# microsoft/UniSpeech

Measured on NVIDIA H100. Metric: audio-sec/sec fwd+bwd, higher is better.
Workload: dtype bf16

## Files before the change

unispeech_b200/csrc/attn_fwd.cu:

```cuda
#include "../../include/unispeech_b200.h"
#include "attn_common.cuh"
#include "common.h"
#include <type_traits>

namespace b200 {

__device__ __forceinline__ float fast_exp2(float x) {
  float y;
  asm("ex2.approx.ftz.f32 %0, %1;" : "=f"(y) : "f"(x));
  return y;
}
__device__ __forceinline__ uint32_t warp_bit_transpose(uint32_t x, int lane) {
#pragma unroll
  for (int s = 16; s >= 1; s >>= 1) {
    const uint32_t m = (s == 16) ? 0x0000FFFFu : (s == 8) ? 0x00FF00FFu : (s == 4) ? 0x0F0F0F0Fu : (s == 2) ? 0x33333333u : 0x55555555u;
    const uint32_t y = __shfl_xor_sync(0xffffffffu, x, s);
    x = (lane & s) ? ((x & ~m) | ((y >> s) & m)) : ((x & m) | ((y << s) & ~m));
  }
  return x;
}
__device__ __forceinline__ void mbar_arrive_rel(uint64_t* bar) {
  asm volatile("mbarrier.arrive.release.cta.shared::cta.b64 _, [%0];" ::"r"(smem_u32(bar)) : "memory");
}

constexpr int kFwdQ = 0;
constexpr int kFwdK = 16384;
constexpr int kFwdV = 32768;
constexpr int kFwdP = 49152;
constexpr int kSPitch = kAttnTile + 4;
constexpr int kFwdS = 81920;
constexpr int kFwdStage = kFwdS + kAttnTile * kSPitch * 4;
constexpr int kFwdThreads = 160;
constexpr int kTabCopies = 4;
constexpr int kTabStride = 2 * kAttnTile + 8;
constexpr int kStageFloats = kTabCopies * kTabStride + kAttnTile + 4;
constexpr int kFwdSmem = kFwdStage + 2 * kStageFloats * 4 + 1024;
constexpr float kRebase = 1.2089258e24f;

__device__ __forceinline__ void lds_row32(const float* src, uint32_t* r) {
#pragma unroll
  for (int i = 0; i < 8; ++i) {
    const float4 v = reinterpret_cast<const float4*>(src)[i];
    r[4 * i] = __float_as_uint(v.x); r[4 * i + 1] = __float_as_uint(v.y);
    r[4 * i + 2] = __float_as_uint(v.z); r[4 * i + 3] = __float_as_uint(v.w);
  }
}

template <bool HAS_BIAS, bool DROP>
__global__ void __launch_bounds__(kFwdThreads, 1) attn_fwd_kernel(const __grid_constant__ CUtensorMap tm,
                                                                 const __grid_constant__ AttnParams p) {
  pdl_grid_sync();
  const int tid = threadIdx.x, warp = tid >> 5, lane = tid & 31;
  const int q0 = blockIdx.x * kAttnTile, h = blockIdx.y, b = blockIdx.z;
  const int T = p.T, D = p.D, N = p.n_tiles;

  extern __shared__ uint8_t smem_raw[];
  uint8_t* smem = smem_raw + ((1024u - (smem_u32(smem_raw) & 1023u)) & 1023u);
  uint8_t* sQ = smem + kFwdQ;
  uint8_t* sK = smem + kFwdK;
  uint8_t* sV = smem + kFwdV;
  uint8_t* sP = smem + kFwdP;
  float* s_f = reinterpret_cast<float*>(smem + kFwdS);
  float* stage = reinterpret_cast<float*>(smem + kFwdStage);

  __shared__ uint64_t q_full, k_full, k_empty, v_full, v_empty, stage_full[2];
  __shared__ float row_scale[kAttnTile];

  __shared__ int n_eff_s, live_s;
  if (tid == 0) { n_eff_s = p.key_pad != nullptr ? 1 : N; live_s = 0; }
  __syncthreads();
  if (p.key_pad != nullptr) {
    int last_valid = -1;
    bool live = false;
    for (int j = tid; j < T; j += kFwdThreads) {
      if (p.key_pad[static_cast<long long>(b) * T + j] == 0) {
        last_valid = j;
        if (j >= q0 && j < q0 + kAttnTile) live = true;
      }
    }
    if (last_valid >= 0) atomicMax(&n_eff_s, last_valid / kAttnTile + 1);
    if (live) live_s = 1;
  }
  __syncthreads();
  const int n_eff = n_eff_s;
  if (p.key_pad != nullptr && live_s == 0) {
    if (tid < kAttnTile && q0 + tid < T) {
      uint4* dst = reinterpret_cast<uint4*>(p.out + (static_cast<long long>(b) * T + q0 + tid) * D + h * kHeadDim);
#pragma unroll
      for (int g = 0; g < 8; ++g) dst[g] = make_uint4(0u, 0u, 0u, 0u);
      if (p.lse != nullptr) p.lse[(static_cast<long long>(b) * p.H + h) * T + q0 + tid] = INFINITY;
    }
    return;
  }

  if (warp == 4 && lane == 0) {
    tma_prefetch_desc(&tm);
    mbar_init(&q_full, 1);
    mbar_init(&k_full, 1);
    mbar_init(&v_full, 1);
    mbar_init(&k_empty, 4);
    mbar_init(&v_empty, 4);
    mbar_init(&stage_full[0], 32);
    mbar_init(&stage_full[1], 32);
    fence_mbar_init();
    mbar_expect_tx(&q_full, 16384);
    tma_load_4d(sQ, &tm, &q_full, h * kHeadDim, q0, b, 0);
    mbar_expect_tx(&k_full, 16384);
    tma_load_4d(sK, &tm, &k_full, D + h * kHeadDim, 0, b, 0);
    mbar_expect_tx(&v_full, 16384);
    tma_load_4d(sV, &tm, &v_full, 2 * D + h * kHeadDim, 0, b, 0);
  }
  __syncthreads();

  if (warp == 4) {
    auto fill_stage = [&](int n) {
      float* stg = stage + (n & 1) * kStageFloats;
      const int k0 = n * kAttnTile;
      if (HAS_BIAS) {
        const int base = k0 + (T - 1) - (q0 + kAttnTile - 1);
        const float* tab_h = p.tab + static_cast<long long>(h) * (2 * T - 1);
        float v[9];
#pragma unroll
        for (int t = 0; t < 9; ++t) {
          const int i = lane + 32 * t, gi = base + i;
          v[t] = (i < 2 * kAttnTile + kTabCopies - 1 && gi >= 0 && gi < 2 * T - 1) ? tab_h[gi] : 0.f;
        }
#pragma unroll
        for (int t = 0; t < 9; ++t)
#pragma unroll
          for (int c = 0; c < kTabCopies; ++c) {
            const int k = lane + 32 * t - c;
            if (k >= 0 && k < 2 * kAttnTile) stg[c * kTabStride + k] = v[t];
          }
      }
      float kb[4];
      int cnt = 0;
#pragma unroll
      for (int e = 0; e < 4; ++e) {
        const int j = k0 + 4 * lane + e;
        const bool masked = (j >= T) || (p.key_pad != nullptr && p.key_pad[static_cast<long long>(b) * T + j] != 0);
        kb[e] = masked ? -INFINITY : 0.f;
        cnt += masked ? 1 : 0;
      }
      reinterpret_cast<float4*>(stg + kTabCopies * kTabStride)[lane] = make_float4(kb[0], kb[1], kb[2], kb[3]);
      cnt = __reduce_add_sync(0xffffffffu, cnt);
      if (lane == 0) reinterpret_cast<int*>(stg)[kTabCopies * kTabStride + kAttnTile] = (cnt == 0) ? 0 : (cnt == kAttnTile ? 2 : 1);
      mbar_arrive(&stage_full[n & 1]);
    };
    fill_stage(0);
    if (n_eff > 1) fill_stage(1);
    for (int n = 1; n < n_eff; ++n) {
      const uint32_t ph = (n - 1) & 1;
      mbar_wait(&k_empty, ph);
      if (lane == 0) {
        mbar_expect_tx(&k_full, 16384);
        tma_load_4d(sK, &tm, &k_full, D + h * kHeadDim, n * kAttnTile, b, 0);
      }
      mbar_wait(&v_empty, ph);
      if (lane == 0) {
        mbar_expect_tx(&v_full, 16384);
        tma_load_4d(sV, &tm, &v_full, 2 * D + h * kHeadDim, n * kAttnTile, b, 0);
      }
      if (n + 1 < n_eff) fill_stage(n + 1);
    }
  } else {
    const int r = tid;
    const bool row_valid = (q0 + r) < T;
    const float* s_row = s_f + r * kSPitch;
    const int fr = 16 * (warp & 3) + (lane >> 2);
    float o_acc[2][32];

    float gl = 0.f;
    if (HAS_BIAS) {
      const float g = (p.gate != nullptr && row_valid) ? p.gate[(static_cast<long long>(b) * p.H + h) * T + q0 + r] : 1.0f;
      gl = g * kLog2e;
    }
    const float sc = p.scale * kLog2e;
    const int toff = kAttnTile - 1 - r;
    const int tab_off = (toff & 3) * kTabStride + (toff & ~3);
    uint32_t rk0 = 0, rk1 = 0;
    uint32_t* mask_row = nullptr;
    if (DROP) {
      const uint32_t rowid = static_cast<uint32_t>(b * p.H + h) * static_cast<uint32_t>(T) + static_cast<uint32_t>(q0 + r);
      rk0 = drop_row_k0(p.drop_k0, rowid);
      rk1 = drop_row_k1(p.drop_k1, rowid);
      mask_row = p.drop_mask + (static_cast<long long>(b * p.H + h) * (4 * N) + ((q0 + r) >> 5)) * (N * kAttnTile);
    }

    float m_ref = -INFINITY, l_run = 0.f;
    mbar_wait(&q_full, 0);

    for (int n = 0; n < n_eff; ++n) {
      const int k0 = n * kAttnTile;
      mbar_wait(&k_full, n & 1);
#pragma unroll 1
      for (int hm = 0; hm < 2; ++hm) {
        float acc[64];
        const uint32_t a = smem_u32(sQ) + hm * 8192, bb = smem_u32(sK);
        wgmma_fence();
#pragma unroll
        for (int k = 0; k < 4; ++k)
          wgmma_m64n128k16<0, 0>(acc, make_smem_desc_sw128(a + k * 32, 16, 1024), make_smem_desc_sw128(bb + k * 32, 16, 1024),
                                 k > 0 ? 1u : 0u);
        wgmma_commit();
        wgmma_wait<0>();
        acc_to_smem<128>(acc, s_f, kSPitch, 64 * hm);
      }
      if (lane == 0) mbar_arrive(&k_empty);
      named_bar_sync(1, kAttnTile);
      mbar_wait(&stage_full[n & 1], (n >> 1) & 1);
      const float* stg = stage + (n & 1) * kStageFloats;
      const float4* tab4 = reinterpret_cast<const float4*>(stg + tab_off);
      const float* kbias = stg + kTabCopies * kTabStride;
      const bool msk = reinterpret_cast<const int*>(stg)[kTabCopies * kTabStride + kAttnTile] != 0;

      auto tile_max = [&]() {
        float mx = -INFINITY;
#pragma unroll 1
        for (int c0 = 0; c0 < kAttnTile; c0 += 32) {
          uint32_t su[32];
          lds_row32(s_row + c0, su);
#pragma unroll
          for (int q = 0; q < 8; ++q) {
            float4 tb = make_float4(0.f, 0.f, 0.f, 0.f);
            if (HAS_BIAS) tb = tab4[c0 / 4 + q];
            float x0 = __uint_as_float(su[4 * q]) * sc, x1 = __uint_as_float(su[4 * q + 1]) * sc;
            float x2 = __uint_as_float(su[4 * q + 2]) * sc, x3 = __uint_as_float(su[4 * q + 3]) * sc;
            if (HAS_BIAS) {
              x0 = fmaf(gl, tb.x, x0); x1 = fmaf(gl, tb.y, x1); x2 = fmaf(gl, tb.z, x2); x3 = fmaf(gl, tb.w, x3);
            }
            if (msk) {
              const float4 kb = *reinterpret_cast<const float4*>(kbias + c0 + 4 * q);
              x0 += kb.x; x1 += kb.y; x2 += kb.z; x3 += kb.w;
            }
            mx = fmaxf(fmaxf(mx, fmaxf(x0, x1)), fmaxf(x2, x3));
          }
        }
        return mx;
      };

      if (__any_sync(0xffffffffu, m_ref == -INFINITY)) {
        const float mx = tile_max();
        if (m_ref == -INFINITY) m_ref = mx;
      }
      auto softmax_tile = [&](auto MSK) -> float {
        constexpr bool kMsk = decltype(MSK)::value;
        const float neg_ref = (m_ref == -INFINITY) ? 0.f : -m_ref;
        float part0 = 0.f, part1 = 0.f, part2 = 0.f, part3 = 0.f;
#pragma unroll 1
        for (int cc = 0; cc < 4; ++cc) {
          const int c0 = cc * 32;
          uint32_t su[32];
          lds_row32(s_row + c0, su);
          float pv[32];
          uint32_t rowbits = 0, hbits = 0;
#pragma unroll
          for (int q = 0; q < 8; ++q) {
            float4 tb = make_float4(0.f, 0.f, 0.f, 0.f), kb = make_float4(0.f, 0.f, 0.f, 0.f);
            if (HAS_BIAS) tb = tab4[c0 / 4 + q];
            if (kMsk) kb = *reinterpret_cast<const float4*>(kbias + c0 + 4 * q);
            const float tbv[4] = {tb.x, tb.y, tb.z, tb.w};
            const float kbv[4] = {kb.x, kb.y, kb.z, kb.w};
#pragma unroll
            for (int e = 0; e < 4; ++e) {
              const int j = 4 * q + e;
              float x = fmaf(__uint_as_float(su[j]), sc, neg_ref);
              if (HAS_BIAS) x = fmaf(gl, tbv[e], x);
              if (kMsk) x += kbv[e];
              const float ex = fast_exp2(x);
              if (e == 0) part0 += ex; else if (e == 1) part1 += ex; else if (e == 2) part2 += ex; else part3 += ex;
              if (DROP) {
                if ((j & 1) == 0) hbits = drop_bits(rk0, rk1, static_cast<uint32_t>(k0 + c0 + j) >> 1);
                const bool keep = (j & 1) ? drop_keep_hi(hbits, p.drop_thr_hi) : drop_keep_lo(hbits, p.drop_thr_hi);
                if (keep) rowbits |= (1u << j);
                pv[j] = keep ? ex : 0.f;
              } else {
                pv[j] = ex;
              }
            }
          }
          if (DROP) {
            const uint32_t mword = warp_bit_transpose(rowbits, lane);
            mask_row[k0 + c0 + lane] = mword;
          }
#pragma unroll
          for (int g = 0; g < 4; ++g) {
            uint4 w;
            w.x = pack_bf16x2(pv[g * 8 + 0], pv[g * 8 + 1]);
            w.y = pack_bf16x2(pv[g * 8 + 2], pv[g * 8 + 3]);
            w.z = pack_bf16x2(pv[g * 8 + 4], pv[g * 8 + 5]);
            w.w = pack_bf16x2(pv[g * 8 + 6], pv[g * 8 + 7]);
            store_sw128_chunk(sP, r, (c0 >> 3) + g, w);
          }
        }
        return (part0 + part1) + (part2 + part3);
      };
      float lsum, fac = 1.0f;
#pragma unroll 1
      while (true) {
        lsum = msk ? softmax_tile(std::true_type{}) : softmax_tile(std::false_type{});
        if (!__any_sync(0xffffffffu, !(lsum < kRebase))) break;
        const float m_new = fmaxf(m_ref, tile_max());
        const float factor = (m_ref == -INFINITY) ? 0.f : fast_exp2(m_ref - m_new);
        fac *= factor;
        l_run *= factor;
        m_ref = m_new;
      }
      l_run += lsum;
      row_scale[r] = fac;

      fence_proxy_async_smem();
      named_bar_sync(1, kAttnTile);
      if (n > 0) {
#pragma unroll
        for (int hm = 0; hm < 2; ++hm) {
          const float f0 = row_scale[64 * hm + fr], f1 = row_scale[64 * hm + fr + 8];
#pragma unroll
          for (int i = 0; i < 32; ++i) o_acc[hm][i] *= ((i >> 1) & 1) ? f1 : f0;
        }
      }
      mbar_wait(&v_full, n & 1);
      const uint32_t bv = smem_u32(sV);
      wgmma_fence();
#pragma unroll
      for (int hm = 0; hm < 2; ++hm) {
        const uint32_t a = smem_u32(sP) + hm * 8192;
#pragma unroll
        for (int k = 0; k < 8; ++k)
          wgmma_m64n64k16<0, 1>(o_acc[hm], make_smem_desc_sw128(a + (k >> 2) * 16384 + (k & 3) * 32, 16, 1024),
                                make_smem_desc_sw128(bv + k * 2048, 8192, 1024), (n > 0 || k > 0) ? 1u : 0u);
      }
      wgmma_commit();
      wgmma_wait<0>();
      if (lane == 0) mbar_arrive(&v_empty);
      named_bar_sync(1, kAttnTile);
    }

    row_scale[r] = l_run > 0.f ? (DROP ? p.drop_rp : 1.0f) / l_run : 0.f;
    if (row_valid && p.lse != nullptr)
      p.lse[(static_cast<long long>(b) * p.H + h) * T + q0 + r] = (l_run > 0.f) ? (m_ref + log2f(l_run)) : INFINITY;
    named_bar_sync(1, kAttnTile);
#pragma unroll
    for (int hm = 0; hm < 2; ++hm) {
#pragma unroll
      for (int rr = 0; rr < 2; ++rr) {
        const int row = 64 * hm + fr + 8 * rr;
        if (q0 + row < T) {
          const float inv = row_scale[row];
          __nv_bfloat16* dst = p.out + (static_cast<long long>(b) * T + q0 + row) * D + h * kHeadDim + 2 * (lane & 3);
#pragma unroll
          for (int g = 0; g < 8; ++g)
            *reinterpret_cast<uint32_t*>(dst + 8 * g) =
                pack_bf16x2(o_acc[hm][4 * g + 2 * rr] * inv, o_acc[hm][4 * g + 2 * rr + 1] * inv);
        }
      }
    }
  }
}

int make_qkv_tmap(CUtensorMap* out, const void* qkv, int T, int B, int D3, int box_rows);

}

using namespace b200;

extern "C" {

int b200s_attn_fwd_dropout(const void* qkv, const float* gate, const float* tab, const uint8_t* key_pad, void* out, float* lse,
                           int B, int T, int H, float scale, float drop_p, uint32_t key0, uint32_t key1, uint32_t* drop_mask,
                           b200s_stream stream) {
  B200_CHECK_ARG(qkv && out, "attn_fwd: null pointer");
  B200_CHECK_ARG(drop_p >= 0.f && drop_p < 1.f, "attn_fwd: dropout p=%f out of range [0,1)", static_cast<double>(drop_p));
  B200_CHECK_ARG(drop_p == 0.f || drop_mask != nullptr, "attn_fwd: dropout needs the mask buffer (b200s_attn_dropout_mask_words)");
  B200_CHECK_ARG(static_cast<long long>(B) * H * T < (1LL << 32), "attn_fwd: B*H*T exceeds the 32-bit dropout row counter");
  const int D = H * kHeadDim;
  CUtensorMap tm;
  AttnParams p;
  memset(&p, 0, sizeof(p));
  p.T = T; p.H = H; p.B = B; p.D = D;
  p.n_tiles = ceil_div(T, kAttnTile);
  B200_CHECK_ARG(T >= 1, "attn_fwd: T=%d out of range", T);
  const int smem = kFwdSmem;
  if (make_qkv_tmap(&tm, qkv, T, B, 3 * D, kAttnTile)) return -3;
  p.scale = scale;
  p.gate = gate; p.tab = tab; p.key_pad = key_pad;
  p.out = static_cast<__nv_bfloat16*>(out);
  p.lse = lse;
  const bool drop = drop_p > 0.f;
  p.drop_mask = drop_mask;
  p.drop_k0 = key0; p.drop_k1 = key1;
  p.drop_thr_hi = drop_threshold16(drop_p) << 16;
  p.drop_rp = 1.0f / (1.0f - drop_p);
  dim3 grid(ceil_div(T, kAttnTile), H, B);
  cudaStream_t st = static_cast<cudaStream_t>(stream);
  void (*kern)(const CUtensorMap, const AttnParams) =
      tab != nullptr ? (drop ? attn_fwd_kernel<true, true> : attn_fwd_kernel<true, false>)
                     : (drop ? attn_fwd_kernel<false, true> : attn_fwd_kernel<false, false>);
  B200_CHECK_CUDA(cudaFuncSetAttribute(kern, cudaFuncAttributeMaxDynamicSharedMemorySize, smem));
  B200_CHECK_CUDA(launch_pdl(kern, dim3(grid), dim3(kFwdThreads), smem, st, tm, p));
  B200_CHECK_LAUNCH();
  return 0;
}

int b200s_attn_fwd(const void* qkv, const float* gate, const float* tab, const uint8_t* key_pad, void* out, float* lse,
                   int B, int T, int H, float scale, b200s_stream stream) {
  return b200s_attn_fwd_dropout(qkv, gate, tab, key_pad, out, lse, B, T, H, scale, 0.f, 0u, 0u, nullptr, stream);
}

long long b200s_attn_dropout_mask_words(int B, int T, int H) { return attn_drop_mask_words(B, H, T); }

}
```

Before: 2505.

## Restructure attention forward into two warpgroups with register softmax and pipelined QK/PV

Replaces the one-warpgroup-plus-producer-warp design with two consumer warpgroups of 128 threads, each owning 64 query rows. The S tile stays in registers instead of round-tripping through shared memory, and P is fed to the PV wgmma from registers. A three-stage K/V TMA ring lets the QK^T of tile n overlap the PV of tile n-1, and bias and mask staging move to per-warpgroup cp.async. This removes the smem S/P traffic and the serialised wgmma waits, at the cost of higher register pressure and a more complex rebase path that recomputes S when the running sum overflows.

```diff
diff --git a/unispeech_b200/csrc/attn_fwd.cu b/unispeech_b200/csrc/attn_fwd.cu
--- a/unispeech_b200/csrc/attn_fwd.cu
+++ b/unispeech_b200/csrc/attn_fwd.cu
@@ -19,32 +19,37 @@
   }
   return x;
 }
-__device__ __forceinline__ void mbar_arrive_rel(uint64_t* bar) {
-  asm volatile("mbarrier.arrive.release.cta.shared::cta.b64 _, [%0];" ::"r"(smem_u32(bar)) : "memory");
-}
-
+__device__ __forceinline__ uint32_t compact_every4(uint32_t x) {
+  x &= 0x11111111u;
+  x = (x | (x >> 3)) & 0x03030303u;
+  x = (x | (x >> 6)) & 0x000F000Fu;
+  return (x | (x >> 12)) & 0xFFu;
+}
+__device__ __forceinline__ bool named_bar_any(int id, int count, bool pred) {
+  uint32_t r;
+  asm volatile(
+      "{\n\t.reg .pred p, q;\n\t"
+      "setp.ne.u32 p, %1, 0;\n\t"
+      "bar.red.or.pred q, %2, %3, p;\n\t"
+      "selp.u32 %0, 1, 0, q;\n\t}"
+      : "=r"(r)
+      : "r"(static_cast<uint32_t>(pred)), "r"(id), "r"(count)
+      : "memory");
+  return r != 0;
+}
+
+constexpr int kFwdStages = 3;
 constexpr int kFwdQ = 0;
 constexpr int kFwdK = 16384;
-constexpr int kFwdV = 32768;
-constexpr int kFwdP = 49152;
-constexpr int kSPitch = kAttnTile + 4;
-constexpr int kFwdS = 81920;
-constexpr int kFwdStage = kFwdS + kAttnTile * kSPitch * 4;
-constexpr int kFwdThreads = 160;
-constexpr int kTabCopies = 4;
-constexpr int kTabStride = 2 * kAttnTile + 8;
-constexpr int kStageFloats = kTabCopies * kTabStride + kAttnTile + 4;
-constexpr int kFwdSmem = kFwdStage + 2 * kStageFloats * 4 + 1024;
+constexpr int kFwdV = kFwdK + kFwdStages * 16384;
+constexpr int kFwdStage = kFwdV + kFwdStages * 16384;
+constexpr int kFwdThreads = 256;
+constexpr int kTabCopies = 2;
+constexpr int kWgWin = 192;
+constexpr int kTabStride = kWgWin + 8;
+constexpr int kStageFloats = kTabCopies * kTabStride + kAttnTile;
+constexpr int kFwdSmem = kFwdStage + 4 * kStageFloats * 4 + 1024;
 constexpr float kRebase = 1.2089258e24f;
-
-__device__ __forceinline__ void lds_row32(const float* src, uint32_t* r) {
-#pragma unroll
-  for (int i = 0; i < 8; ++i) {
-    const float4 v = reinterpret_cast<const float4*>(src)[i];
-    r[4 * i] = __float_as_uint(v.x); r[4 * i + 1] = __float_as_uint(v.y);
-    r[4 * i + 2] = __float_as_uint(v.z); r[4 * i + 3] = __float_as_uint(v.w);
-  }
-}
 
 template <bool HAS_BIAS, bool DROP>
 __global__ void __launch_bounds__(kFwdThreads, 1) attn_fwd_kernel(const __grid_constant__ CUtensorMap tm,
@@ -59,12 +64,9 @@
   uint8_t* sQ = smem + kFwdQ;
   uint8_t* sK = smem + kFwdK;
   uint8_t* sV = smem + kFwdV;
-  uint8_t* sP = smem + kFwdP;
-  float* s_f = reinterpret_cast<float*>(smem + kFwdS);
   float* stage = reinterpret_cast<float*>(smem + kFwdStage);
 
-  __shared__ uint64_t q_full, k_full, k_empty, v_full, v_empty, stage_full[2];
-  __shared__ float row_scale[kAttnTile];
+  __shared__ uint64_t q_full, k_full[kFwdStages], k_empty[kFwdStages], v_full[kFwdStages], v_empty[kFwdStages];
 
   __shared__ int n_eff_s, live_s;
   if (tid == 0) { n_eff_s = p.key_pad != nullptr ? 1 : N; live_s = 0; }
@@ -93,268 +95,284 @@
     return;
   }
 
-  if (warp == 4 && lane == 0) {
+  if (tid == 0) {
     tma_prefetch_desc(&tm);
     mbar_init(&q_full, 1);
-    mbar_init(&k_full, 1);
-    mbar_init(&v_full, 1);
-    mbar_init(&k_empty, 4);
-    mbar_init(&v_empty, 4);
-    mbar_init(&stage_full[0], 32);
-    mbar_init(&stage_full[1], 32);
+#pragma unroll
+    for (int s = 0; s < kFwdStages; ++s) {
+      mbar_init(&k_full[s], 1);
+      mbar_init(&v_full[s], 1);
+      mbar_init(&k_empty[s], 8);
+      mbar_init(&v_empty[s], 8);
+    }
     fence_mbar_init();
     mbar_expect_tx(&q_full, 16384);
     tma_load_4d(sQ, &tm, &q_full, h * kHeadDim, q0, b, 0);
-    mbar_expect_tx(&k_full, 16384);
-    tma_load_4d(sK, &tm, &k_full, D + h * kHeadDim, 0, b, 0);
-    mbar_expect_tx(&v_full, 16384);
-    tma_load_4d(sV, &tm, &v_full, 2 * D + h * kHeadDim, 0, b, 0);
+    for (int n = 0; n < 2 && n < n_eff; ++n) {
+      mbar_expect_tx(&k_full[n], 16384);
+      tma_load_4d(sK + n * 16384, &tm, &k_full[n], D + h * kHeadDim, n * kAttnTile, b, 0);
+      mbar_expect_tx(&v_full[n], 16384);
+      tma_load_4d(sV + n * 16384, &tm, &v_full[n], 2 * D + h * kHeadDim, n * kAttnTile, b, 0);
+    }
   }
   __syncthreads();
 
-  if (warp == 4) {
-    auto fill_stage = [&](int n) {
-      float* stg = stage + (n & 1) * kStageFloats;
-      const int k0 = n * kAttnTile;
-      if (HAS_BIAS) {
-        const int base = k0 + (T - 1) - (q0 + kAttnTile - 1);
-        const float* tab_h = p.tab + static_cast<long long>(h) * (2 * T - 1);
-        float v[9];
-#pragma unroll
-        for (int t = 0; t < 9; ++t) {
-          const int i = lane + 32 * t, gi = base + i;
-          v[t] = (i < 2 * kAttnTile + kTabCopies - 1 && gi >= 0 && gi < 2 * T - 1) ? tab_h[gi] : 0.f;
+  const int c = warp >> 2, w = warp & 3, qd = lane & 3;
+  const int r0 = 64 * c + 16 * w + (lane >> 2);
+  const float sc = p.scale * kLog2e;
+  float gl[2] = {0.f, 0.f};
+  uint32_t rk0[2] = {0u, 0u}, rk1[2] = {0u, 0u};
+#pragma unroll
+  for (int hh = 0; hh < 2; ++hh) {
+    const int row = q0 + r0 + 8 * hh;
+    if (HAS_BIAS) {
+      const float g = (p.gate != nullptr && row < T) ? p.gate[(static_cast<long long>(b) * p.H + h) * T + row] : 1.0f;
+      gl[hh] = g * kLog2e;
+    }
+    if (DROP) {
+      const uint32_t rowid = static_cast<uint32_t>(b * p.H + h) * static_cast<uint32_t>(T) + static_cast<uint32_t>(row);
+      rk0[hh] = drop_row_k0(p.drop_k0, rowid);
+      rk1[hh] = drop_row_k1(p.drop_k1, rowid);
+    }
+  }
+  float* const wg_stage = stage + 2 * c * kStageFloats;
+  const int t = tid & 127;
+  const float* tab_h = HAS_BIAS ? p.tab + static_cast<long long>(h) * (2 * T - 1) : nullptr;
+  auto fill_bias = [&](int n) {
+    float* stg = wg_stage + (n & 1) * kStageFloats;
+    const int gbase = n * kAttnTile + T - 64 - 64 * c - q0;
+#pragma unroll
+    for (int u = 0; u < 3; ++u) {
+      const int e = (t + 128 * u) / kWgWin, i = (t + 128 * u) % kWgWin, gi = gbase + i + e;
+      const bool ok = gi >= 0 && gi < 2 * T - 1;
+      cp_async_4_zfill(stg + e * kTabStride + i, tab_h + (ok ? gi : 0), ok);
+    }
+    cp_async_commit();
+  };
+  auto key_masked = [&](int n) {
+    const int j = n * kAttnTile + t;
+    return j >= T || (p.key_pad != nullptr && p.key_pad[static_cast<long long>(b) * T + j] != 0);
+  };
+  const int tbase = 63 + 64 * c - r0 + 2 * qd;
+  const int tab_off = (tbase & 1) * kTabStride + (tbase & ~1);
+  uint16_t* mask_half = nullptr;
+  if (DROP)
+    mask_half = reinterpret_cast<uint16_t*>(p.drop_mask + (static_cast<long long>(b * p.H + h) * (4 * N) + (q0 >> 5) + 2 * c + (w >> 1)) *
+                                                              (N * kAttnTile)) + (w & 1);
+
+  float s[64];
+  float o[32];
+  uint32_t pr[32];
+#pragma unroll
+  for (int i = 0; i < 32; ++i) o[i] = 0.f;
+  float m_ref[2] = {-INFINITY, -INFINITY}, l_run[2] = {0.f, 0.f};
+  const uint32_t qa = smem_u32(sQ) + c * 8192;
+
+  auto issue_s = [&](int n) {
+    const uint32_t kb = smem_u32(sK) + (n % kFwdStages) * 16384;
+#pragma unroll
+    for (int k = 0; k < 4; ++k)
+      wgmma_m64n128k16<0, 0>(s, make_smem_desc_sw128(qa + k * 32, 16, 1024), make_smem_desc_sw128(kb + k * 32, 16, 1024),
+                             k > 0 ? 1u : 0u);
+  };
+  auto issue_pv = [&](int n) {
+    const uint32_t vb = smem_u32(sV) + (n % kFwdStages) * 16384;
+#pragma unroll
+    for (int k = 0; k < 8; ++k) wgmma_m64n64k16_rs<1>(o, pr + 4 * k, make_smem_desc_sw128(vb + k * 2048, 8192, 1024), 1u);
+  };
+
+  auto refill = [&](int n, uint64_t* empty, uint64_t* full, uint8_t* ring, int col) {
+    if (tid == 0 && n + 2 < n_eff) {
+      const int slot = (n + 2) % kFwdStages;
+      if (n > 0) mbar_wait(&empty[slot], ((n - 1) / kFwdStages) & 1);
+      mbar_expect_tx(&full[slot], 16384);
+      tma_load_4d(ring + slot * 16384, &tm, &full[slot], col + h * kHeadDim, (n + 2) * kAttnTile, b, 0);
+    }
+  };
+  float o_fac[2] = {1.f, 1.f};
+  bool rebased = false;
+  bool km = false;
+  auto softmax_step = [&](int n) {
+    const int k0 = n * kAttnTile;
+    if (HAS_BIAS) cp_async_wait_all();
+    const bool msk = named_bar_any(1 + c, 128, km);
+    bool km_next = false;
+    if (n + 1 < n_eff) {
+      if (HAS_BIAS) fill_bias(n + 1);
+      km_next = key_masked(n + 1);
+    }
+    const float* stg = wg_stage + (n & 1) * kStageFloats;
+    const float* tabp = stg + tab_off;
+    const float* kbias = stg + kTabCopies * kTabStride + 2 * qd;
+
+    auto tile_max = [&](float (&mx)[2]) {
+      mx[0] = mx[1] = -INFINITY;
+#pragma unroll
+      for (int g = 0; g < 16; ++g) {
+        const float2 kb = msk ? *reinterpret_cast<const float2*>(kbias + 8 * g) : make_float2(0.f, 0.f);
+#pragma unroll
+        for (int hh = 0; hh < 2; ++hh) {
+          float2 tb = make_float2(0.f, 0.f);
+          if (HAS_BIAS) tb = *reinterpret_cast<const float2*>(tabp + 8 * (g - hh));
+          float x0 = s[4 * g + 2 * hh] * sc, x1 = s[4 * g + 2 * hh + 1] * sc;
+          if (HAS_BIAS) { x0 = fmaf(gl[hh], tb.x, x0); x1 = fmaf(gl[hh], tb.y, x1); }
+          if (msk) { x0 += kb.x; x1 += kb.y; }
+          mx[hh] = fmaxf(mx[hh], fmaxf(x0, x1));
         }
-#pragma unroll
-        for (int t = 0; t < 9; ++t)
-#pragma unroll
-          for (int c = 0; c < kTabCopies; ++c) {
-            const int k = lane + 32 * t - c;
-            if (k >= 0 && k < 2 * kAttnTile) stg[c * kTabStride + k] = v[t];
-          }
-      }
-      float kb[4];
-      int cnt = 0;
-#pragma unroll
-      for (int e = 0; e < 4; ++e) {
-        const int j = k0 + 4 * lane + e;
-        const bool masked = (j >= T) || (p.key_pad != nullptr && p.key_pad[static_cast<long long>(b) * T + j] != 0);
-        kb[e] = masked ? -INFINITY : 0.f;
-        cnt += masked ? 1 : 0;
-      }
-      reinterpret_cast<float4*>(stg + kTabCopies * kTabStride)[lane] = make_float4(kb[0], kb[1], kb[2], kb[3]);
-      cnt = __reduce_add_sync(0xffffffffu, cnt);
-      if (lane == 0) reinterpret_cast<int*>(stg)[kTabCopies * kTabStride + kAttnTile] = (cnt == 0) ? 0 : (cnt == kAttnTile ? 2 : 1);
-      mbar_arrive(&stage_full[n & 1]);
+      }
+#pragma unroll
+      for (int hh = 0; hh < 2; ++hh) {
+        mx[hh] = fmaxf(mx[hh], __shfl_xor_sync(0xffffffffu, mx[hh], 1));
+        mx[hh] = fmaxf(mx[hh], __shfl_xor_sync(0xffffffffu, mx[hh], 2));
+      }
     };
-    fill_stage(0);
-    if (n_eff > 1) fill_stage(1);
-    for (int n = 1; n < n_eff; ++n) {
-      const uint32_t ph = (n - 1) & 1;
-      mbar_wait(&k_empty, ph);
-      if (lane == 0) {
-        mbar_expect_tx(&k_full, 16384);
-        tma_load_4d(sK, &tm, &k_full, D + h * kHeadDim, n * kAttnTile, b, 0);
-      }
-      mbar_wait(&v_empty, ph);
-      if (lane == 0) {
-        mbar_expect_tx(&v_full, 16384);
-        tma_load_4d(sV, &tm, &v_full, 2 * D + h * kHeadDim, n * kAttnTile, b, 0);
-      }
-      if (n + 1 < n_eff) fill_stage(n + 1);
-    }
-  } else {
-    const int r = tid;
-    const bool row_valid = (q0 + r) < T;
-    const float* s_row = s_f + r * kSPitch;
-    const int fr = 16 * (warp & 3) + (lane >> 2);
-    float o_acc[2][32];
-
-    float gl = 0.f;
-    if (HAS_BIAS) {
-      const float g = (p.gate != nullptr && row_valid) ? p.gate[(static_cast<long long>(b) * p.H + h) * T + q0 + r] : 1.0f;
-      gl = g * kLog2e;
-    }
-    const float sc = p.scale * kLog2e;
-    const int toff = kAttnTile - 1 - r;
-    const int tab_off = (toff & 3) * kTabStride + (toff & ~3);
-    uint32_t rk0 = 0, rk1 = 0;
-    uint32_t* mask_row = nullptr;
-    if (DROP) {
-      const uint32_t rowid = static_cast<uint32_t>(b * p.H + h) * static_cast<uint32_t>(T) + static_cast<uint32_t>(q0 + r);
-      rk0 = drop_row_k0(p.drop_k0, rowid);
-      rk1 = drop_row_k1(p.drop_k1, rowid);
-      mask_row = p.drop_mask + (static_cast<long long>(b * p.H + h) * (4 * N) + ((q0 + r) >> 5)) * (N * kAttnTile);
-    }
-
-    float m_ref = -INFINITY, l_run = 0.f;
-    mbar_wait(&q_full, 0);
-
-    for (int n = 0; n < n_eff; ++n) {
-      const int k0 = n * kAttnTile;
-      mbar_wait(&k_full, n & 1);
-#pragma unroll 1
-      for (int hm = 0; hm < 2; ++hm) {
-        float acc[64];
-        const uint32_t a = smem_u32(sQ) + hm * 8192, bb = smem_u32(sK);
-        wgmma_fence();
-#pragma unroll
-        for (int k = 0; k < 4; ++k)
-          wgmma_m64n128k16<0, 0>(acc, make_smem_desc_sw128(a + k * 32, 16, 1024), make_smem_desc_sw128(bb + k * 32, 16, 1024),
-                                 k > 0 ? 1u : 0u);
-        wgmma_commit();
-        wgmma_wait<0>();
-        acc_to_smem<128>(acc, s_f, kSPitch, 64 * hm);
-      }
-      if (lane == 0) mbar_arrive(&k_empty);
-      named_bar_sync(1, kAttnTile);
-      mbar_wait(&stage_full[n & 1], (n >> 1) & 1);
-      const float* stg = stage + (n & 1) * kStageFloats;
-      const float4* tab4 = reinterpret_cast<const float4*>(stg + tab_off);
-      const float* kbias = stg + kTabCopies * kTabStride;
-      const bool msk = reinterpret_cast<const int*>(stg)[kTabCopies * kTabStride + kAttnTile] != 0;
-
-      auto tile_max = [&]() {
-        float mx = -INFINITY;
-#pragma unroll 1
-        for (int c0 = 0; c0 < kAttnTile; c0 += 32) {
-          uint32_t su[32];
-          lds_row32(s_row + c0, su);
-#pragma unroll
-          for (int q = 0; q < 8; ++q) {
-            float4 tb = make_float4(0.f, 0.f, 0.f, 0.f);
-            if (HAS_BIAS) tb = tab4[c0 / 4 + q];
-            float x0 = __uint_as_float(su[4 * q]) * sc, x1 = __uint_as_float(su[4 * q + 1]) * sc;
-            float x2 = __uint_as_float(su[4 * q + 2]) * sc, x3 = __uint_as_float(su[4 * q + 3]) * sc;
-            if (HAS_BIAS) {
-              x0 = fmaf(gl, tb.x, x0); x1 = fmaf(gl, tb.y, x1); x2 = fmaf(gl, tb.z, x2); x3 = fmaf(gl, tb.w, x3);
+    if (__any_sync(0xffffffffu, m_ref[0] == -INFINITY || m_ref[1] == -INFINITY)) {
+      float mx[2];
+      tile_max(mx);
+#pragma unroll
+      for (int hh = 0; hh < 2; ++hh)
+        if (m_ref[hh] == -INFINITY) m_ref[hh] = mx[hh];
+    }
+    uint32_t rowbits[2];
+    auto softmax_tile = [&](auto MSK, float (&lsum)[2]) {
+      constexpr bool kMsk = decltype(MSK)::value;
+      float part[2][2] = {{0.f, 0.f}, {0.f, 0.f}};
+      rowbits[0] = rowbits[1] = 0u;
+#pragma unroll
+      for (int g = 0; g < 16; ++g) {
+        float2 kb = make_float2(0.f, 0.f);
+        if (kMsk) kb = *reinterpret_cast<const float2*>(kbias + 8 * g);
+#pragma unroll
+        for (int hh = 0; hh < 2; ++hh) {
+          const float neg_ref = (m_ref[hh] == -INFINITY) ? 0.f : -m_ref[hh];
+          float2 tb = make_float2(0.f, 0.f);
+          if (HAS_BIAS) tb = *reinterpret_cast<const float2*>(tabp + 8 * (g - hh));
+          const float tbv[2] = {tb.x, tb.y}, kbv[2] = {kb.x, kb.y};
+          uint32_t hbits = 0u;
+          if (DROP) hbits = drop_bits(rk0[hh], rk1[hh], static_cast<uint32_t>(k0 + 8 * g + 2 * qd) >> 1);
+#pragma unroll
+          for (int e = 0; e < 2; ++e) {
+            const int i = 4 * g + 2 * hh + e;
+            float x = fmaf(s[i], sc, neg_ref);
+            if (HAS_BIAS) x = fmaf(gl[hh], tbv[e], x);
+            if (kMsk) x += kbv[e];
+            const float ex = fast_exp2(x);
+            part[hh][e] += ex;
+            if (DROP) {
+              const bool keep = e ? drop_keep_hi(hbits, p.drop_thr_hi) : drop_keep_lo(hbits, p.drop_thr_hi);
+              if (keep) rowbits[hh] |= 1u << (2 * g + e);
+              s[i] = keep ? ex : 0.f;
+            } else {
+              s[i] = ex;
             }
-            if (msk) {
-              const float4 kb = *reinterpret_cast<const float4*>(kbias + c0 + 4 * q);
-              x0 += kb.x; x1 += kb.y; x2 += kb.z; x3 += kb.w;
-            }
-            mx = fmaxf(fmaxf(mx, fmaxf(x0, x1)), fmaxf(x2, x3));
           }
         }
-        return mx;
-      };
-
-      if (__any_sync(0xffffffffu, m_ref == -INFINITY)) {
-        const float mx = tile_max();
-        if (m_ref == -INFINITY) m_ref = mx;
-      }
-      auto softmax_tile = [&](auto MSK) -> float {
-        constexpr bool kMsk = decltype(MSK)::value;
-        const float neg_ref = (m_ref == -INFINITY) ? 0.f : -m_ref;
-        float part0 = 0.f, part1 = 0.f, part2 = 0.f, part3 = 0.f;
-#pragma unroll 1
-        for (int cc = 0; cc < 4; ++cc) {
-          const int c0 = cc * 32;
-          uint32_t su[32];
-          lds_row32(s_row + c0, su);
-          float pv[32];
-          uint32_t rowbits = 0, hbits = 0;
-#pragma unroll
-          for (int q = 0; q < 8; ++q) {
-            float4 tb = make_float4(0.f, 0.f, 0.f, 0.f), kb = make_float4(0.f, 0.f, 0.f, 0.f);
-            if (HAS_BIAS) tb = tab4[c0 / 4 + q];
-            if (kMsk) kb = *reinterpret_cast<const float4*>(kbias + c0 + 4 * q);
-            const float tbv[4] = {tb.x, tb.y, tb.z, tb.w};
-            const float kbv[4] = {kb.x, kb.y, kb.z, kb.w};
-#pragma unroll
-            for (int e = 0; e < 4; ++e) {
-              const int j = 4 * q + e;
-              float x = fmaf(__uint_as_float(su[j]), sc, neg_ref);
-              if (HAS_BIAS) x = fmaf(gl, tbv[e], x);
-              if (kMsk) x += kbv[e];
-              const float ex = fast_exp2(x);
-              if (e == 0) part0 += ex; else if (e == 1) part1 += ex; else if (e == 2) part2 += ex; else part3 += ex;
-              if (DROP) {
-                if ((j & 1) == 0) hbits = drop_bits(rk0, rk1, static_cast<uint32_t>(k0 + c0 + j) >> 1);
-                const bool keep = (j & 1) ? drop_keep_hi(hbits, p.drop_thr_hi) : drop_keep_lo(hbits, p.drop_thr_hi);
-                if (keep) rowbits |= (1u << j);
-                pv[j] = keep ? ex : 0.f;
-              } else {
-                pv[j] = ex;
-              }
-            }
-          }
-          if (DROP) {
-            const uint32_t mword = warp_bit_transpose(rowbits, lane);
-            mask_row[k0 + c0 + lane] = mword;
-          }
-#pragma unroll
-          for (int g = 0; g < 4; ++g) {
-            uint4 w;
-            w.x = pack_bf16x2(pv[g * 8 + 0], pv[g * 8 + 1]);
-            w.y = pack_bf16x2(pv[g * 8 + 2], pv[g * 8 + 3]);
-            w.z = pack_bf16x2(pv[g * 8 + 4], pv[g * 8 + 5]);
-            w.w = pack_bf16x2(pv[g * 8 + 6], pv[g * 8 + 7]);
-            store_sw128_chunk(sP, r, (c0 >> 3) + g, w);
-          }
-        }
-        return (part0 + part1) + (part2 + part3);
-      };
-      float lsum, fac = 1.0f;
-#pragma unroll 1
-      while (true) {
-        lsum = msk ? softmax_tile(std::true_type{}) : softmax_tile(std::false_type{});
-        if (!__any_sync(0xffffffffu, !(lsum < kRebase))) break;
-        const float m_new = fmaxf(m_ref, tile_max());
-        const float factor = (m_ref == -INFINITY) ? 0.f : fast_exp2(m_ref - m_new);
-        fac *= factor;
-        l_run *= factor;
-        m_ref = m_new;
-      }
-      l_run += lsum;
-      row_scale[r] = fac;
-
-      fence_proxy_async_smem();
-      named_bar_sync(1, kAttnTile);
-      if (n > 0) {
-#pragma unroll
-        for (int hm = 0; hm < 2; ++hm) {
-          const float f0 = row_scale[64 * hm + fr], f1 = row_scale[64 * hm + fr + 8];
-#pragma unroll
-          for (int i = 0; i < 32; ++i) o_acc[hm][i] *= ((i >> 1) & 1) ? f1 : f0;
-        }
-      }
-      mbar_wait(&v_full, n & 1);
-      const uint32_t bv = smem_u32(sV);
+      }
+#pragma unroll
+      for (int hh = 0; hh < 2; ++hh) {
+        float v = part[hh][0] + part[hh][1];
+        v += __shfl_xor_sync(0xffffffffu, v, 1);
+        v += __shfl_xor_sync(0xffffffffu, v, 2);
+        lsum[hh] = v;
+      }
+    };
+    float lsum[2];
+    if (msk) softmax_tile(std::true_type{}, lsum); else softmax_tile(std::false_type{}, lsum);
+    bool need[2] = {!(lsum[0] < kRebase), !(lsum[1] < kRebase)};
+    if (named_bar_any(1 + c, 128, need[0] || need[1])) {
+      wgmma_wait<0>();
       wgmma_fence();
-#pragma unroll
-      for (int hm = 0; hm < 2; ++hm) {
-        const uint32_t a = smem_u32(sP) + hm * 8192;
-#pragma unroll
-        for (int k = 0; k < 8; ++k)
-          wgmma_m64n64k16<0, 1>(o_acc[hm], make_smem_desc_sw128(a + (k >> 2) * 16384 + (k & 3) * 32, 16, 1024),
-                                make_smem_desc_sw128(bv + k * 2048, 8192, 1024), (n > 0 || k > 0) ? 1u : 0u);
-      }
+      issue_s(n);
       wgmma_commit();
       wgmma_wait<0>();
-      if (lane == 0) mbar_arrive(&v_empty);
-      named_bar_sync(1, kAttnTile);
-    }
-
-    row_scale[r] = l_run > 0.f ? (DROP ? p.drop_rp : 1.0f) / l_run : 0.f;
-    if (row_valid && p.lse != nullptr)
-      p.lse[(static_cast<long long>(b) * p.H + h) * T + q0 + r] = (l_run > 0.f) ? (m_ref + log2f(l_run)) : INFINITY;
-    named_bar_sync(1, kAttnTile);
-#pragma unroll
-    for (int hm = 0; hm < 2; ++hm) {
-#pragma unroll
-      for (int rr = 0; rr < 2; ++rr) {
-        const int row = 64 * hm + fr + 8 * rr;
-        if (q0 + row < T) {
-          const float inv = row_scale[row];
-          __nv_bfloat16* dst = p.out + (static_cast<long long>(b) * T + q0 + row) * D + h * kHeadDim + 2 * (lane & 3);
-#pragma unroll
-          for (int g = 0; g < 8; ++g)
-            *reinterpret_cast<uint32_t*>(dst + 8 * g) =
-                pack_bf16x2(o_acc[hm][4 * g + 2 * rr] * inv, o_acc[hm][4 * g + 2 * rr + 1] * inv);
-        }
-      }
-    }
+      float mx[2];
+      tile_max(mx);
+      rebased = true;
+#pragma unroll
+      for (int hh = 0; hh < 2; ++hh) {
+        if (!need[hh]) continue;
+        const float m_new = fmaxf(m_ref[hh], mx[hh]);
+        const float factor = (m_ref[hh] == -INFINITY) ? 0.f : fast_exp2(m_ref[hh] - m_new);
+        l_run[hh] *= factor;
+        o_fac[hh] = factor;
+        m_ref[hh] = m_new;
+      }
+      if (msk) softmax_tile(std::true_type{}, lsum); else softmax_tile(std::false_type{}, lsum);
+    }
+    l_run[0] += lsum[0];
+    l_run[1] += lsum[1];
+    if (lane == 0) mbar_arrive(&k_empty[n % kFwdStages]);
+    refill(n, k_empty, k_full, sK, D);
+
+    if (DROP) {
+      const uint32_t t0 = warp_bit_transpose(rowbits[0], lane), t1 = warp_bit_transpose(rowbits[1], lane);
+      const int col = k0 + 8 * (lane >> 1) + (lane & 1);
+#pragma unroll
+      for (int q = 0; q < 4; ++q)
+        mask_half[2 * (col + 2 * q)] = static_cast<uint16_t>(compact_every4(t0 >> q) | (compact_every4(t1 >> q) << 8));
+    }
+    if (n + 1 < n_eff) wg_stage[((n + 1) & 1) * kStageFloats + kTabCopies * kTabStride + t] = km_next ? -INFINITY : 0.f;
+    km = km_next;
+  };
+  auto apply_rebase = [&]() {
+    if (rebased) {
+#pragma unroll
+      for (int i = 0; i < 32; ++i) o[i] *= o_fac[(i >> 1) & 1];
+      o_fac[0] = o_fac[1] = 1.f;
+      rebased = false;
+    }
+  };
+  auto pack_p = [&]() {
+#pragma unroll
+    for (int m = 0; m < 32; ++m) pr[m] = pack_bf16x2(s[2 * m], s[2 * m + 1]);
+  };
+
+  if (HAS_BIAS) fill_bias(0);
+  km = key_masked(0);
+  wg_stage[kTabCopies * kTabStride + t] = km ? -INFINITY : 0.f;
+  mbar_wait(&q_full, 0);
+  mbar_wait(&k_full[0], 0);
+  wgmma_fence();
+  issue_s(0);
+  wgmma_commit();
+  wgmma_wait<0>();
+  softmax_step(0);
+  refill(0, v_empty, v_full, sV, 2 * D);
+  apply_rebase();
+  pack_p();
+  for (int n = 1; n < n_eff; ++n) {
+    mbar_wait(&k_full[n % kFwdStages], (n / kFwdStages) & 1);
+    mbar_wait(&v_full[(n - 1) % kFwdStages], ((n - 1) / kFwdStages) & 1);
+    wgmma_fence();
+    issue_s(n);
+    wgmma_commit();
+    issue_pv(n - 1);
+    wgmma_commit();
+    wgmma_wait<1>();
+    softmax_step(n);
+    wgmma_wait<0>();
+    if (lane == 0) mbar_arrive(&v_empty[(n - 1) % kFwdStages]);
+    refill(n, v_empty, v_full, sV, 2 * D);
+    apply_rebase();
+    pack_p();
+  }
+  mbar_wait(&v_full[(n_eff - 1) % kFwdStages], ((n_eff - 1) / kFwdStages) & 1);
+  wgmma_fence();
+  issue_pv(n_eff - 1);
+  wgmma_commit();
+  wgmma_wait<0>();
+
+#pragma unroll
+  for (int hh = 0; hh < 2; ++hh) {
+    const int row = q0 + r0 + 8 * hh;
+    if (row >= T) continue;
+    if (qd == 0 && p.lse != nullptr)
+      p.lse[(static_cast<long long>(b) * p.H + h) * T + row] = (l_run[hh] > 0.f) ? (m_ref[hh] + log2f(l_run[hh])) : INFINITY;
+    const float inv = l_run[hh] > 0.f ? (DROP ? p.drop_rp : 1.0f) / l_run[hh] : 0.f;
+    __nv_bfloat16* dst = p.out + (static_cast<long long>(b) * T + row) * D + h * kHeadDim + 2 * qd;
+#pragma unroll
+    for (int g = 0; g < 8; ++g)
+      *reinterpret_cast<uint32_t*>(dst + 8 * g) = pack_bf16x2(o[4 * g + 2 * hh] * inv, o[4 * g + 2 * hh + 1] * inv);
   }
 }
 
```

Result: faster. 2571 (median of 6 runs) (+2.6%).
